# akamiru/bce

Hardware: AMD Instinct MI355X
Metric: MB/s compressed (higher is better)
Workload: dtype u8/u32 integer

## Files before the change

### bce_amd/csrc/host_coder.cpp

```cpp
#include "host_coder.h"

#include "bce_core.h"

#include <stdio.h>
#include <stdlib.h>
#include <string.h>

#include <chrono>
#include <thread>

namespace bce {

const uint8_t kDefaultConfig[9][32] = {
    {0, 0, 5, 5, 5, 4, 4, 4, 4, 4, 4, 4, 4, 4, 4, 4, 4, 4, 4, 4, 4, 4, 4, 4, 4, 4, 4, 4, 4, 4, 4, 0},
    {0, 0, 5, 5, 5, 4, 4, 4, 4, 4, 4, 4, 4, 4, 4, 4, 4, 4, 4, 4, 4, 4, 4, 4, 4, 4, 4, 4, 4, 4, 4, 0},
    {0, 0, 5, 5, 5, 4, 4, 4, 4, 4, 4, 4, 4, 4, 4, 4, 4, 4, 4, 4, 4, 4, 4, 4, 4, 4, 4, 3, 3, 3, 3, 0},
    {0, 0, 5, 5, 5, 4, 4, 4, 4, 4, 4, 4, 4, 4, 4, 4, 4, 4, 4, 4, 4, 4, 3, 3, 3, 3, 3, 3, 3, 3, 3, 0},
    {0, 0, 5, 5, 4, 4, 4, 4, 4, 4, 4, 4, 3, 3, 3, 3, 3, 3, 3, 3, 3, 3, 3, 3, 3, 3, 3, 3, 3, 3, 3, 0},
    {0, 0, 5, 5, 4, 4, 4, 4, 4, 4, 4, 4, 3, 3, 3, 3, 3, 3, 3, 3, 3, 3, 3, 3, 3, 3, 3, 3, 3, 3, 3, 0},
    {0, 0, 5, 4, 4, 4, 4, 4, 4, 3, 3, 3, 3, 3, 3, 3, 3, 3, 3, 3, 3, 3, 3, 3, 3, 3, 3, 3, 3, 3, 3, 0},
    {0, 0, 4, 4, 4, 4, 3, 3, 3, 3, 3, 3, 3, 3, 3, 3, 3, 3, 3, 3, 3, 3, 3, 3, 3, 2, 2, 2, 2, 2, 2, 0},
    {0, 0, 0, 0, 0, 0, 0, 0, 0, 0, 0, 0, 0, 0, 0, 0, 0, 0, 0, 0, 0, 0, 0, 0, 0, 0, 0, 0, 0, 0, 0, 0}};

void RangeCoder::setv(uint32_t s) {
  while (s) { uniform(s & 1, 3); s >>= 1; }
  uniform(2, 3);
}

void RangeCoder::preamble(const uint8_t row[32]) {
  uint32_t last = 0;
  for (int b = 0; b < 32; ++b) {
    const uint32_t bit = row[b];
    uniform(bit != last, 2);
    if (bit != last) uniform(bit, 6);
    last = bit;
  }
}

void RangeCoder::flush() {
  while (!((h_ ^ l_) >> 48)) {
    data_.push_back((uint16_t)(h_ >> 48));
    l_ = (l_ << 16) + 0x0000;
    h_ = (h_ << 16) + 0xFFFF;
  }
  const uint32_t bits = (uint32_t)__builtin_clzll(l_ ^ h_) + 1;
  data_.push_back((uint16_t)((h_ >> (64 - bits)) << (16 - bits)));
}

void HostCoder::begin(const uint8_t config[9][32], const uint32_t C[8], uint32_t n) {
  drain();
  failed_.store(false);
  for (int i = 0; i < 8; ++i) {
    w_[i].busy = 0; w_[i].nsym = 0;
    plane[i] = RangeCoder();
    plane[i].preamble(config[i]);
    plane[i].uniform(C[i], n + 1);
  }
}

const Recip *recip_table() {
  static const std::vector<Recip> tab = [] {
    std::vector<Recip> t(kRecipMax);
    t[0] = t[1] = Recip{0, -1, 0};
    for (uint32_t d = 2; d < kRecipMax; ++d) {
      uint32_t L = 0;
      while ((2ull << L) <= d) ++L;
      if ((d & (d - 1)) == 0) { t[d] = Recip{1ull << (64 - L), -1, 0}; continue; }
      const unsigned __int128 two_s = (unsigned __int128)1 << (64 + L);
      const uint64_t m_dn = (uint64_t)(two_s / d);
      const uint64_t e_dn = (uint64_t)(two_s - (unsigned __int128)m_dn * d);
      const uint64_t e_up = d - e_dn;
      if (e_up <= (1ull << L)) t[d] = Recip{m_dn + 1, -1, L};
      else t[d] = Recip{m_dn, 0, L};
    }
    return t;
  }();
  return tab.data();
}

uint64_t bce_test_div_recip(uint64_t x, uint32_t d) {
  return x == ~0ull ? x / d : div_recip1(x + 1, recip_table()[d]);
}

void RangeCoder::encode_run(const uint64_t *out, uint64_t begin, uint64_t end) {
  const Recip *rt = recip_table();
  uint64_t l = l_, R = h_ - l_ + 1;
  uint16_t stage[64];
  uint32_t ns = 0;
#define BCE_EMIT(v)                                                                                       \
  do {                                                                                                    \
    stage[ns++] = (uint16_t)(v);                                                                          \
    if (__builtin_expect(ns == 64, 0)) { data_.insert(data_.end(), stage, stage + 64); ns = 0; }          \
  } while (0)
#define BCE_STEP(cum, freq, total)                                                                        \
  do {                                                                                                    \
    const uint32_t t_ = (total);                                                                          \
    if (__builtin_expect(R - 1 < t_, 0)) {                                                  \
      for (int i_ = 0; i_ < 4; ++i_) BCE_EMIT(l >> (48 - 16 * i_));                                       \
      l = 0; R = 0;                                                                                       \
    }                                                                                                     \
    const uint64_t step_ =                                                                                \
        (__builtin_expect(R == 0, 0) || t_ >= kRecipMax) ? (R - 1) / t_ : div_recip1(R, rt[t_]);          \
    l += step_ * (cum);                                                                         \
    R = step_ * (freq);                                                \
    while (__builtin_expect(!(((l + R - 1) ^ l) >> 48), 0)) {                     \
      BCE_EMIT((l + R - 1) >> 48);                                                                        \
      l <<= 16;                                                                                           \
      R <<= 16;                                                             \
    }                                                                                                     \
  } while (0)
#define BCE_BIT(bit)                                                                                      \
  do {                                                                                                    \
    if (__builtin_expect(R - 1 < 2u, 0)) {                                                  \
      for (int i_ = 0; i_ < 4; ++i_) BCE_EMIT(l >> (48 - 16 * i_));                                       \
      l = 0; R = 0;                                                                                       \
    }                                                                                                     \
    const uint64_t step_ = (R - 1) >> 1;                                                                  \
    l += step_ & (0ull - (uint64_t)(bit));                                                                \
    R = step_;                                                                                            \
    while (__builtin_expect(!(((l + R - 1) ^ l) >> 48), 0)) {                                             \
      BCE_EMIT((l + R - 1) >> 48);                                                                        \
      l <<= 16;                                                                                           \
      R <<= 16;                                                                                           \
    }                                                                                                     \
  } while (0)
  for (uint64_t i = begin; i < end; ++i) {
    const uint64_t o = out[i];
    uint32_t es = out_esc_sentinel(o);
    if (__builtin_expect(es != 1u, 0))
      for (; es > 1u; es >>= 1) BCE_BIT(es & 1u);
    BCE_STEP(out_cum(o), out_freq(o), out_total(o));
  }
#undef BCE_BIT
#undef BCE_STEP
#undef BCE_EMIT
  data_.insert(data_.end(), stage, stage + ns);
  l_ = l; h_ = l + R - 1;
}

void HostCoder::consume(int p, const SymRun *runs, size_t nruns, const uint64_t *out) {
  RangeCoder &rc = plane[p];
  for (size_t r = 0; r < nruns; ++r) rc.encode_run(out, runs[r].start, runs[r].start + runs[r].count);
}

HostCoder::HostCoder() {
  try {
    for (int p = 0; p < 8; ++p) w_[p].th = std::thread([this, p]() { run(p); });
  } catch (...) {
    stop_threads();
    throw;
  }
}

void HostCoder::stop_threads() {
  for (int p = 0; p < 8; ++p) {
    { std::lock_guard<std::mutex> g(w_[p].mu); w_[p].stop = true; }
    w_[p].cv.notify_all();
  }
  for (int p = 0; p < 8; ++p) if (w_[p].th.joinable()) w_[p].th.join();
}

HostCoder::~HostCoder() { stop_threads(); }

void HostCoder::run(int p) {
  Worker &w = w_[p];
  for (;;) {
    CoderBatch *b = nullptr;
    {
      std::unique_lock<std::mutex> lk(w.mu);
      w.cv.wait(lk, [&] { return w.stop || !w.q.empty(); });
      if (w.q.empty()) return;
      b = w.q.front();
      w.q.pop_front();
    }
    const auto t0 = std::chrono::steady_clock::now();
    try {
      if (b->wait_ready) b->wait_ready();
      if (!failed_.load(std::memory_order_relaxed) && ((plane_mask >> p) & 1u)) {
        consume(p, b->runs[p].data(), b->runs[p].size(), b->out);
        for (const SymRun &r : b->runs[p]) w.nsym += r.count;
      }
    } catch (...) {
      failed_.store(true);
    }
    const double dt = std::chrono::duration<double>(std::chrono::steady_clock::now() - t0).count();
    {
      std::lock_guard<std::mutex> g(done_mu_);
      w.busy += dt;
      b->pending.fetch_sub(1);
      ++completed_;
    }
    done_cv_.notify_all();
  }
}

void HostCoder::submit(CoderBatch *b) {
  b->pending.store(8);
  { std::lock_guard<std::mutex> g(done_mu_); submitted_ += 8; }
  for (int p = 0; p < 8; ++p) {
    { std::lock_guard<std::mutex> g(w_[p].mu); w_[p].q.push_back(b); }
    w_[p].cv.notify_one();
  }
}

void HostCoder::wait(CoderBatch *b) {
  std::unique_lock<std::mutex> lk(done_mu_);
  done_cv_.wait(lk, [&] { return b->pending.load() == 0; });
}

void HostCoder::drain() {
  std::unique_lock<std::mutex> lk(done_mu_);
  done_cv_.wait(lk, [&] { return completed_ == submitted_; });
}

double HostCoder::busy_seconds() {
  std::lock_guard<std::mutex> g(done_mu_);
  double m = 0;
  for (int p = 0; p < 8; ++p) m = w_[p].busy > m ? w_[p].busy : m;
  return m;
}

void HostCoder::finish(const uint8_t config[9][32], uint32_t n, uint32_t offset) {
  if (getenv("BCE_HIP_CODER_DEBUG"))
    for (int p = 0; p < 8; ++p) fprintf(stderr, "coder %d: busy %.1f ms, %llu symbols, %zu words\n", p, w_[p].busy * 1e3, (unsigned long long)w_[p].nsym, plane[p].data().size());
  for (int i = 0; i < 8; ++i) plane[i].flush();
  rebuild_header(config, n, offset);
}

void HostCoder::rebuild_header(const uint8_t config[9][32], uint32_t n, uint32_t offset) {
  unsigned size = 0u;
  for (int i = 0; i < 8; ++i) size += (unsigned)plane[i].data().size();
  RangeCoder mainc;
  mainc.preamble(config[8]);
  mainc.setv(n);
  mainc.uniform(offset, n + 1);
  mainc.setv(size);
  int s = (int)size;
  for (int i = 0; i < 7; ++i) {
    mainc.uniform((uint32_t)plane[i].data().size(), (uint32_t)s + 1);
    s -= (int)plane[i].data().size();
  }
  mainc.flush();
  header_ = mainc.data();
}

size_t HostCoder::archive_words() const {
  size_t w = 1 + header_.size();
  for (int i = 0; i < 8; ++i) w += plane[i].data().size();
  return w;
}

void HostCoder::assemble(uint16_t *dst) const {
  *dst++ = (uint16_t)header_.size();
  memcpy(dst, header_.data(), header_.size() * 2);
  dst += header_.size();
  uint16_t *at[8];
  for (int i = 0; i < 8; ++i) { at[i] = dst; dst += plane[i].data().size(); }
  size_t total = 0;
  for (int i = 0; i < 8; ++i) total += plane[i].data().size();
  if (total < (1u << 20)) {
    for (int i = 0; i < 8; ++i) memcpy(at[i], plane[i].data().data(), plane[i].data().size() * 2);
    return;
  }
  std::thread th[8];
  int started = 0;
  try {
    for (; started < 8; ++started) {
      const int i = started;
      th[i] = std::thread([this, i, &at] { memcpy(at[i], plane[i].data().data(), plane[i].data().size() * 2); });
    }
  } catch (...) {
  }
  for (int i = started; i < 8; ++i) memcpy(at[i], plane[i].data().data(), plane[i].data().size() * 2);
  for (int i = 0; i < started; ++i) th[i].join();
}

void HostCoder::finish(const uint8_t config[9][32], uint32_t n, uint32_t offset, std::vector<uint16_t> &archive) {
  finish(config, n, offset);
  archive.resize(archive_words());
  assemble(archive.data());
}

}
```

### bce_amd/csrc/host_coder.h

```cpp
#pragma once
#include <stddef.h>
#include <stdint.h>

#include <atomic>
#include <condition_variable>
#include <deque>
#include <functional>
#include <mutex>
#include <thread>
#include <vector>

namespace bce {

class alignas(128) RangeCoder {
 public:
  RangeCoder() : l_(0), h_(~0ull) {}
  inline void encode(uint32_t cum, uint32_t freq, uint32_t total) {
    if (__builtin_expect(h_ - l_ < total, 0)) {
      for (int i = 0; i < 4; ++i) data_.push_back((uint16_t)(l_ >> (48 - 16 * i)));
      l_ = 0; h_ = ~0ull;
    }
    const uint64_t step = (h_ - l_) / total;
    l_ += step * cum;
    h_ = l_ + step * freq - 1;
    while (!((h_ ^ l_) >> 48)) {
      data_.push_back((uint16_t)(h_ >> 48));
      l_ = (l_ << 16) + 0x0000;
      h_ = (h_ << 16) + 0xFFFF;
    }
  }
  inline void uniform(uint32_t s, uint32_t k) { encode(s, 1, k); }
  void setv(uint32_t s);
  void preamble(const uint8_t row[32]);
  void flush();
  const std::vector<uint16_t> &data() const { return data_; }
  std::vector<uint16_t> &data() { return data_; }
  void encode_run(const uint64_t *out, uint64_t begin, uint64_t end);

 private:
  uint64_t l_, h_;
  std::vector<uint16_t> data_;
};

struct SymRun { uint64_t start; uint32_t count; uint32_t round; };

struct CoderBatch {
  const uint64_t *out = nullptr;
  std::function<void()> wait_ready;
  std::vector<SymRun> runs[8];
  std::atomic<int> pending{0};
};

struct HostCoder {
  RangeCoder plane[8];
  uint32_t plane_mask = 0xFFu;
  void set_stream(int p, const uint16_t *words, size_t n) { plane[p].data().assign(words, words + n); }
  void rebuild_header(const uint8_t config[9][32], uint32_t n, uint32_t offset);
  HostCoder();
  ~HostCoder();
  void begin(const uint8_t config[9][32], const uint32_t C[8], uint32_t n);
  void consume(int p, const SymRun *runs, size_t nruns, const uint64_t *out);
  void submit(CoderBatch *b);
  void wait(CoderBatch *b);
  void drain();
  void finish(const uint8_t config[9][32], uint32_t n, uint32_t offset);
  size_t archive_words() const;
  void assemble(uint16_t *dst) const;
  void finish(const uint8_t config[9][32], uint32_t n, uint32_t offset, std::vector<uint16_t> &archive);
  double busy_seconds();
  bool failed() const { return failed_.load(); }

 private:
  struct Worker {
    std::thread th;
    std::mutex mu;
    std::condition_variable cv;
    std::deque<CoderBatch *> q;
    double busy = 0;
    uint64_t nsym = 0;
    bool stop = false;
  };
  Worker w_[8];
  std::mutex done_mu_;
  std::condition_variable done_cv_;
  std::vector<uint16_t> header_;
  uint64_t submitted_ = 0, completed_ = 0;
  std::atomic<bool> failed_{false};
  void run(int p);
  void stop_threads();
};

struct Recip { uint64_t m; int32_t am1; uint32_t sh; };
constexpr uint32_t kRecipMax = 8192;
const Recip *recip_table();
inline uint64_t div_recip1(uint64_t x1, const Recip &r) {
  return (uint64_t)(((unsigned __int128)r.m * (x1 + (uint64_t)(int64_t)r.am1)) >> 64) >> r.sh;
}
inline uint64_t div_small(uint64_t x, uint32_t d, const Recip *rt) {
  return (x == ~0ull || d >= kRecipMax) ? x / d : div_recip1(x + 1, rt[d]);
}

extern const uint8_t kDefaultConfig[9][32];
uint64_t bce_test_div_recip(uint64_t x, uint32_t d);

}
```

Before: 824.4.

## Derive range-coder step from previous step via precomputed freq/total ratio table

Adds a ratio table holding 1/t as fixed-point, and computes the next step as mulhi(previous freq * ratio(t), previous step). This exploits that R equals the previous step times the previous freq, shifted together with R. A remainder check falls back to the exact reciprocal division when the estimate is off, and a miss counter plus a test hook are added. The aim is to shorten the serial dependency chain per symbol in the host-side encoder, at the cost of extra multiplies, a table lookup and a possible mispredicted repair branch.

```diff
diff --git a/bce_amd/csrc/host_coder.cpp b/bce_amd/csrc/host_coder.cpp
--- a/bce_amd/csrc/host_coder.cpp
+++ b/bce_amd/csrc/host_coder.cpp
@@ -82,9 +82,25 @@
   return x == ~0ull ? x / d : div_recip1(x + 1, recip_table()[d]);
 }
 
+const Ratio *ratio_table() {
+  static const std::vector<Ratio> tab = [] {
+    std::vector<Ratio> t(kRecipMax, Ratio{0, 0});
+    for (uint32_t d = 2; d < kRecipMax; ++d) {
+      const unsigned __int128 one = (unsigned __int128)1 << 64;
+      const uint64_t m = (uint64_t)(one / d), e = (uint64_t)(one % d);
+      t[d] = e ? Ratio{m, (uint64_t)(((unsigned __int128)e << 64) / d) >> 9} : Ratio{m - 1, ~0ull >> 9};
+    }
+    return t;
+  }();
+  return tab.data();
+}
+
 void RangeCoder::encode_run(const uint64_t *out, uint64_t begin, uint64_t end) {
   const Recip *rt = recip_table();
+  const Ratio *qt = ratio_table();
   uint64_t l = l_, R = h_ - l_ + 1;
+  uint64_t q = 0, miss = 0;
+  uint32_t fp = ~0u;
   uint16_t stage[64];
   uint32_t ns = 0;
 #define BCE_EMIT(v)                                                                                       \
@@ -92,22 +108,38 @@
     stage[ns++] = (uint16_t)(v);                                                                          \
     if (__builtin_expect(ns == 64, 0)) { data_.insert(data_.end(), stage, stage + 64); ns = 0; }          \
   } while (0)
+#define BCE_SHIFT_OUT()                                                                                   \
+  while (__builtin_expect(!(((l + R - 1) ^ l) >> 48), 0)) {                       \
+    BCE_EMIT((l + R - 1) >> 48);                                                                          \
+    l <<= 16;                                                                                             \
+    R <<= 16;                                                               \
+    q <<= 16;                                            \
+  }
 #define BCE_STEP(cum, freq, total)                                                                        \
   do {                                                                                                    \
     const uint32_t t_ = (total);                                                                          \
-    if (__builtin_expect(R - 1 < t_, 0)) {                                                  \
-      for (int i_ = 0; i_ < 4; ++i_) BCE_EMIT(l >> (48 - 16 * i_));                                       \
-      l = 0; R = 0;                                                                                       \
+    uint64_t step_;                                                                                       \
+    if (__builtin_expect(R <= t_, 0)) {                  \
+      if (R) {                                                                                            \
+        for (int i_ = 0; i_ < 4; ++i_) BCE_EMIT(l >> (48 - 16 * i_));                                     \
+        l = 0;                                                                                            \
+      }                                                                                                   \
+      step_ = ~0ull / t_;                                         \
+    } else if (__builtin_expect(fp >= t_ || t_ >= kRecipMax, 0)) {                                        \
+      step_ = t_ >= kRecipMax ? (R - 1) / t_ : div_recip1(R, rt[t_]);                                     \
+    } else {                                                                                              \
+      step_ = mulhi64(ratio_below(fp, qt[t_]), q);                             \
+      if (__builtin_expect((R - 1) - step_ * t_ >= t_, 0)) {                                              \
+        step_ = div_recip1(R, rt[t_]);                                                                    \
+        ++miss;                                                                                           \
+        __asm__ volatile("" : "+r"(step_));              \
+      }                                                                                                   \
     }                                                                                                     \
-    const uint64_t step_ =                                                                                \
-        (__builtin_expect(R == 0, 0) || t_ >= kRecipMax) ? (R - 1) / t_ : div_recip1(R, rt[t_]);          \
     l += step_ * (cum);                                                                         \
     R = step_ * (freq);                                                \
-    while (__builtin_expect(!(((l + R - 1) ^ l) >> 48), 0)) {                     \
-      BCE_EMIT((l + R - 1) >> 48);                                                                        \
-      l <<= 16;                                                                                           \
-      R <<= 16;                                                             \
-    }                                                                                                     \
+    q = step_;                                                                                            \
+    fp = (freq);                                                                                          \
+    BCE_SHIFT_OUT();                                                                                      \
   } while (0)
 #define BCE_BIT(bit)                                                                                      \
   do {                                                                                                    \
@@ -118,14 +150,12 @@
     const uint64_t step_ = (R - 1) >> 1;                                                                  \
     l += step_ & (0ull - (uint64_t)(bit));                                                                \
     R = step_;                                                                                            \
-    while (__builtin_expect(!(((l + R - 1) ^ l) >> 48), 0)) {                                             \
-      BCE_EMIT((l + R - 1) >> 48);                                                                        \
-      l <<= 16;                                                                                           \
-      R <<= 16;                                                                                           \
-    }                                                                                                     \
+    q = step_;                                                                                            \
+    fp = 1u;                                                                                              \
+    BCE_SHIFT_OUT();                                                                                      \
   } while (0)
-  for (uint64_t i = begin; i < end; ++i) {
-    const uint64_t o = out[i];
+  for (const uint64_t *rec = out + begin, *const rec_end = out + end; rec != rec_end; ++rec) {
+    const uint64_t o = *rec;
     uint32_t es = out_esc_sentinel(o);
     if (__builtin_expect(es != 1u, 0))
       for (; es > 1u; es >>= 1) BCE_BIT(es & 1u);
@@ -133,9 +163,21 @@
   }
 #undef BCE_BIT
 #undef BCE_STEP
+#undef BCE_SHIFT_OUT
 #undef BCE_EMIT
   data_.insert(data_.end(), stage, stage + ns);
   l_ = l; h_ = l + R - 1;
+  misses_ += miss;
+}
+
+uint64_t bce_test_encode_run(const uint64_t *rec, const uint32_t *run_len, size_t nruns, uint64_t *l, uint64_t *h,
+                             std::vector<uint16_t> &words) {
+  RangeCoder rc(*l, *h);
+  uint64_t at = 0;
+  for (size_t r = 0; r < nruns; ++r) { rc.encode_run(rec, at, at + run_len[r]); at += run_len[r]; }
+  words.insert(words.end(), rc.data().begin(), rc.data().end());
+  *l = rc.low(); *h = rc.high();
+  return rc.misses();
 }
 
 void HostCoder::consume(int p, const SymRun *runs, size_t nruns, const uint64_t *out) {
@@ -222,7 +264,7 @@
 
 void HostCoder::finish(const uint8_t config[9][32], uint32_t n, uint32_t offset) {
   if (getenv("BCE_HIP_CODER_DEBUG"))
-    for (int p = 0; p < 8; ++p) fprintf(stderr, "coder %d: busy %.1f ms, %llu symbols, %zu words\n", p, w_[p].busy * 1e3, (unsigned long long)w_[p].nsym, plane[p].data().size());
+    for (int p = 0; p < 8; ++p) fprintf(stderr, "coder %d: busy %.1f ms, %llu symbols, %zu words, %llu repaired quotients\n", p, w_[p].busy * 1e3, (unsigned long long)w_[p].nsym, plane[p].data().size(), (unsigned long long)plane[p].misses());
   for (int i = 0; i < 8; ++i) plane[i].flush();
   rebuild_header(config, n, offset);
 }
diff --git a/bce_amd/csrc/host_coder.h b/bce_amd/csrc/host_coder.h
--- a/bce_amd/csrc/host_coder.h
+++ b/bce_amd/csrc/host_coder.h
@@ -15,6 +15,7 @@
 class alignas(128) RangeCoder {
  public:
   RangeCoder() : l_(0), h_(~0ull) {}
+  RangeCoder(uint64_t l, uint64_t h) : l_(l), h_(h) {}
   inline void encode(uint32_t cum, uint32_t freq, uint32_t total) {
     if (__builtin_expect(h_ - l_ < total, 0)) {
       for (int i = 0; i < 4; ++i) data_.push_back((uint16_t)(l_ >> (48 - 16 * i)));
@@ -36,9 +37,13 @@
   const std::vector<uint16_t> &data() const { return data_; }
   std::vector<uint16_t> &data() { return data_; }
   void encode_run(const uint64_t *out, uint64_t begin, uint64_t end);
+  uint64_t low() const { return l_; }
+  uint64_t high() const { return h_; }
+  uint64_t misses() const { return misses_; }
 
  private:
   uint64_t l_, h_;
+  uint64_t misses_ = 0;
   std::vector<uint16_t> data_;
 };
 
@@ -100,7 +105,15 @@
   return (x == ~0ull || d >= kRecipMax) ? x / d : div_recip1(x + 1, rt[d]);
 }
 
+
+struct Ratio { uint64_t m, r2; };
+const Ratio *ratio_table();
+inline uint64_t mulhi64(uint64_t a, uint64_t b) { return (uint64_t)(((unsigned __int128)a * b) >> 64); }
+inline uint64_t ratio_below(uint32_t f, const Ratio &r) { return (uint64_t)f * r.m + (((uint64_t)f * r.r2) >> 55); }
+
 extern const uint8_t kDefaultConfig[9][32];
 uint64_t bce_test_div_recip(uint64_t x, uint32_t d);
+uint64_t bce_test_encode_run(const uint64_t *rec, const uint32_t *run_len, size_t nruns, uint64_t *l, uint64_t *h,
+                             std::vector<uint16_t> &words);
 
 }
```

After: 729.0. 11.6% lower.
